# cchao0116/EasyDGL

Hardware: AMD Instinct MI355X
Metric: sequences/sec (fwd+bwd+Adam) B=512 L=100 d=128 |I|=20K (higher is better)
Workload: dtype bf16

## Files before the change

### easydgl_amd/_lib.py

```python
from __future__ import annotations

import ctypes
import os
from ctypes import c_char_p, c_float, c_int, c_int64, c_long, c_uint32, c_void_p

import torch

_HERE = os.path.dirname(os.path.abspath(__file__))
LIB_PATH = os.environ.get("EDGL_LIB_PATH") or os.path.join(_HERE, "libeasydgl_hip.so")

F32, BF16 = 0, 1
EPI_BIAS, EPI_GELU, EPI_SAVE_PRE, EPI_MUL_DGELU, EPI_ACCUM, EPI_OUT_F32, EPI_RELU = 1, 2, 4, 8, 16, 32, 64
MAU_CAUSAL, MAU_NO_DIAG, MAU_DIAG_ZERO = 1, 2, 4
MAU_NO_SKIP = 8
MAU_STREAM = 16
TATTN_CAUSAL = 1

P, I, F, L, U32, I64 = c_void_p, c_int, c_float, c_long, c_uint32, c_int64

SIGNATURES = {
    "edgl_last_error": (c_char_p, []),
    "edgl_version": (I, []),
    "edgl_profile_next": (I, [I, P, P]),
    "edgl_rng_advance": (I, [P, P]),
# ... 52 lines not shown
    "edgl_scatter_rows": (I, [P, P, I, I, P, I, P]),
    "edgl_score_lse_fwd": (I, [P, P, P, P, I, I, I, I, I, P, P, P, P, P, I, P]),
    "edgl_ce_loss_fwd": (I, [P, P, P, I, P, P, P]),
    "edgl_ce_loss_fwd_add": (I, [P, P, P, I, P, P, P, P, P]),
    "edgl_ce_loss_fwd_add_w": (I, [P, P, P, I, P, P, P, P, P, P]),
    "edgl_score_bwd_workspace": (L, [I, I, I, I, I]),
    "edgl_score_ce_bwd": (I, [P, P, P, P, P, P, P, I, I, I, I, I, P, P, P, P, P, I, P]),
    "edgl_score_flash_workspace": (L, [I, I, I, I, I]),
    "edgl_score_flash_fwd": (I, [P, P, P, P, I, I, I, I, I, P, P, P, P, I, P]),
    "edgl_score_prepare_table": (I, [P, I, I, I, I, I, P, I, P]),
    "edgl_score_flash_fwd_pre": (I, [P, P, P, P, I, I, I, I, I, P, P, P, P, I, I, P]),
    "edgl_score_flash_fwd_coef": (I, [P, P, P, P, I, I, I, P, P, P, P, P, I, P]),
    "edgl_score_flash_fwd_coef_w": (I, [P, P, P, P, I, I, I, P, P, P, P, P, P, I, P]),
    "edgl_score_flash_fwd_rows_w": (I, [P, P, P, P, I, I, I, P, P, P, P, P, P, P, P, I, P]),
    "edgl_score_ce_nparts": (I, [I, I]),
    "edgl_score_flash_fwd_rows_wp": (I, [P, P, P, P, I, I, I, P, P, P, P, P, P, P, P, P, I, P]),
    "edgl_ce_loss_parts": (I, [P, I, P, P, P, P, P]),
    "edgl_score_flash_bwd": (I, [P, P, P, P, P, P, P, I, I, I, I, I, P, P, P, P, P, I, P]),
    "edgl_score_flash_bwd_ex": (I, [P, P, P, P, P, P, P, I, I, I, I, I, P, P, P, P, P, I, I, P]),
    "edgl_score_flash_label_term": (I, [P, P, P, P, I, I, I, I, I, P, P, P, I, P]),
    "edgl_score_flash_label_term_det": (I, [P, P, P, P, I, I, I, I, I, P, P, P, P, I, P]),
    "edgl_reduce_defer": (I, [I, P]),
    "edgl_reduce_flush": (I, [P]),
    "edgl_mask_topk": (I, [P, I, I, I, P, I, I, P, P, P]),
    "edgl_score_topk_fused_supported": (I, [I, I, I, I, I, I]),
    "edgl_score_topk_fused_workspace": (L, [I, I, I, I, I]),
    "edgl_score_topk_fused": (I, [P, P, P, P, I, I, I, I, I, I, I, P, P, P, I, P]),
    "edgl_topk_merge": (I, [P, P, I, I, I, P, P, P]),
    "edgl_rank_metrics": (I, [P, I, I, P, P, P]),
    "edgl_tpp_workspace": (I, []),
    "edgl_tpp_fwd": (I, [P, P, P, P, P, I, I, I, I, I, F, P, P, I, P]),
    "edgl_tpp_bwd": (I, [P, P, P, P, P, I, I, I, I, I, F, P, P, P, P]),
    "edgl_tpp_fwd_bwd": (I, [P, P, P, P, P, I, I, I, I, I, F, P, P, I, P, P]),
    "edgl_tpp_norm": (I, [P, P, I, I, I, P, P]),
    "edgl_tpp_fwd_bwd_ex": (I, [P, P, P, P, P, I, I, I, I, I, F, P, P, I, P, I, P]),
    "edgl_tpp_rows_workspace": (L, [I, I, I]),
    "edgl_tpp_fwd_bwd_rows": (I, [P, P, P, P, P, I, I, I, I, I, F, P, P, I, P, P]),
    "edgl_tpp_prep_bytes": (L, [I, I, I]),
    "edgl_tpp_prep": (I, [P, P, P, P, I, I, I, I, P, P]),
    "edgl_bimau_bwd_tpp": (I, [P, P, P, P, P, P, P, I, P, F, P, P, P, I, I, I, I, I, F, P, U32, P, F, P, P, P, P, P, P, I, I, P]),
    "edgl_tpp_finish_parts": (I, [P, I, F, I, P, I, I, I, P, P, I, P]),
    "edgl_tpp_finish_parts_n": (I, [P, I, F, I, P, P, I, P]),
    "edgl_dp_counts": (I, [P, P, I, I, I, P, P]),
    "edgl_adam_step": (I, [P, P, P, P, L, F, F, F, F, P, F, P, I, P, P]),
    "edgl_step_begin": (I, [P, P, F, F, F, P]),
    "edgl_adam_apply": (I, [P, P, P, P, L, F, F, F, P, F, P, I, P, P]),
# ... 124 lines not shown
```

### easydgl_amd/build.py

```python
from __future__ import annotations

import hashlib
import os
import subprocess
import sys
from concurrent.futures import ThreadPoolExecutor

HERE = os.path.dirname(os.path.abspath(__file__))
CSRC = os.path.join(HERE, "csrc")
OUT = os.path.join(HERE, "libeasydgl_hip.so")
SOURCES = ["k_misc.hip", "k_data.hip", "k_encode.hip", "k_gemm.hip", "k_gemm2.hip", "k_layernorm.hip", "k_bimau_fwd.hip", "k_bimau_bwd.hip", "k_bimau_big.hip", "k_bimau_stream.hip",
           "k_score.hip", "k_score_strip.hip", "k_score_stripw.hip", "k_eval_topk.hip", "k_tattn.hip", "k_coding.hip", "k_tail.hip", "k_segsum.hip"]
HEADERS = ["edgl_common.h", "batch_prep.h", "score_plan.h", "topk_select.h", "gemm_tile.h", "bimau_common.h", "bimau_fwd_impl.h", "bimau_bwd_impl.h", os.path.join("..", "..", "include", "easydgl_hip.h")]
FLAGS = ["--offload-arch=gfx950", "-O3", "-std=c++17", "-fPIC", "-munsafe-fp-atomics", "-Wno-unused-result"]
EXTRA_FLAGS = {"k_bimau_fwd.hip": ["-mllvm", "-amdgpu-mfma-vgpr-form=1"],
               "k_bimau_bwd.hip": ["-mllvm", "-amdgpu-mfma-vgpr-form=1"],
               "k_bimau_big.hip": ["-mllvm", "-amdgpu-mfma-vgpr-form=1"],
               "k_bimau_stream.hip": ["-mllvm", "-amdgpu-mfma-vgpr-form=1"],
               "k_tattn.hip": ["-mllvm", "-amdgpu-mfma-vgpr-form=1"],
               "k_score_strip.hip": ["-fno-slp-vectorize", "-Wno-unused-value"] + (["-DSTRIP_SAFE"] if os.environ.get("EDGL_STRIP_SAFE") else []),
               "k_score_stripw.hip": ["-fno-slp-vectorize", "-Wno-unused-value"] + (["-DSTRIP_SAFE"] if os.environ.get("EDGL_STRIP_SAFE") else [])}


def _hipcc() -> str:
    for c in (os.environ.get("HIPCC"), "/opt/rocm/bin/hipcc", "hipcc"):
        if c and (os.path.isabs(c) and os.path.exists(c) or not os.path.isabs(c)):
            return c
    raise RuntimeError("hipcc not found")


def _digest(paths, extra=()) -> str:
    h = hashlib.sha256()
    for e in extra:
        h.update(str(e).encode() + b"\0")
    for p in paths:
        with open(p, "rb") as f:
# ... 56 lines not shown
```

### easydgl_amd/csrc/k_encode.hip

```cpp
#include "edgl_common.h"
#include "batch_prep.h"

namespace {

struct EncP {
    const int64_t* ids; const float* ts; const void* item_tab; const float* pos_tab; const float* mark_emb;
    const uint8_t* mark_table; const float* tscale;
    int B, T, C, E, I; int64_t mask_id; float time_scale;
    float rate; const uint64_t* rng; uint32_t stream_id;
    void* x0; float* spans; uint8_t* marks;
    int dhp, dht; float sq;
};

template <typename T>
__device__ __forceinline__ void encode_fwd_block(const EncP& p, long block) {
    const int cpr = p.C >> 3;
    const long gid = block * blockDim.x + threadIdx.x;
    const long row = gid / cpr;
    if (row >= (long)p.B * p.T) return;
    const int cv = (int)(gid % cpr), c0 = cv * 8, j0 = c0 >> 1;
    const int t = (int)(row % p.T);
    const int64_t id = p.ids[row];
    const int t1 = (t == 0) ? 1 : t;
    const long r1 = p.T > 1 ? row - t + t1 : row + 1;
// ... 96 lines not shown
};
template <typename T>
__global__ __launch_bounds__(256) void encode_prep_kernel(EncP p, PrepP q) {
    extern __shared__ __attribute__((aligned(16))) char prep_smem[];
    const int bid = (int)blockIdx.x;
    if (bid == 0) {
        batch_prep::compact_scan_body<256>(q.labels, q.R, q.perm, q.inv, q.nvalid, q.labels_c, reinterpret_cast<int*>(prep_smem));
    } else if (bid < q.nprep) {
        batch_prep::tpp_prep_sample(q.mpos, q.labels, q.ts_raw, p.mark_table, p.B, p.T, q.M, q.desc, bid - 1, prep_smem);
    } else {
        encode_fwd_block<T>(p, (long)(bid - q.nprep));
    }
}

struct EncBwdP {
    const int64_t* ids; const uint8_t* marks; const void* dx0;
    int B, T, C, E, I; float rate; const uint64_t* rng; uint32_t stream_id;
    float* d_item; float* part_pos; float* part_mk; int nchunk;
    int srows;
    const void* add1; const void* add2;
    float sq;
    const void* lab_rows; const int64_t* lab_ids; const float* lab_coef; const int32_t* lab_nvalid; int lab_R; int lab_blk0;
    float* d_bias;
    float* d_mark_zero;
};

template <typename T>
__global__ __launch_bounds__(256) void encode_bwd_kernel(EncBwdP p) {
    extern __shared__ float sm[];
    __shared__ float s_nm[64];
    const int t = blockIdx.x, chunk = blockIdx.y;
    if (t == 0 && chunk == 0 && p.d_mark_zero)
        for (int i = threadIdx.x; i < p.E * p.C; i += blockDim.x) p.d_mark_zero[i] = 0.f;
    const int bper = (p.B + p.nchunk - 1) / p.nchunk;
    const int b0 = chunk * bper, b1 = min(p.B, b0 + bper);
    const int cpr = p.C / 4, rows_par = 256 / cpr;
    const int cv = threadIdx.x % cpr, rl = threadIdx.x / cpr, c0 = cv * 4;
    const bool on = threadIdx.x < rows_par * cpr;
    const DropKey dk = make_dropkey(p.rng, p.stream_id, p.rate);
    float apos[4] = {0.f, 0.f, 0.f, 0.f}, amk[4] = {0.f, 0.f, 0.f, 0.f};
    for (int bb = b0; bb < b1; bb += 64) {
        __syncthreads();
        if (threadIdx.x < 64 && bb + threadIdx.x < b1) {
            const uint8_t* mrow = p.marks + ((long)(bb + threadIdx.x) * p.T + t) * p.E;
            int nm = 0;
            for (int e = 0; e < p.E; ++e) nm += mrow[e];
// ... 105 lines not shown
            float gv[4];
#pragma unroll
            for (int j = 0; j < 4; ++j) gv[j] = to_f32(g0.v[j]);
            drop_apply4(dk, (uint64_t)row * 3 * p.C + c0, gv);
#pragma unroll
            for (int j = 0; j < 4; ++j) atomicAdd(dst + j, sq * gv[j]);
        }
    }
    __syncthreads();
    for (int i = tid; i < SR * p.C; i += 256) {
        const int r = i / p.C, c = i % p.C;
        if (s_lead[r] == r && s_id[r] != 0) atomicAdd(p.d_item + (long)s_id[r] * p.C + c, acc[i]);
    }
}

typedef __attribute__((ext_vector_type(4))) short enc_s16x4;
__device__ __forceinline__ uint2 enc_tr_read(const bf16* tile, int ld, int k0, int z0, int lane) {
    const int G = lane >> 4, s = lane & 15;
    const bf16* p = tile + (k0 + 4 * G + (s >> 2)) * ld + z0 + 4 * (s & 3);
    enc_s16x4 v = __builtin_amdgcn_ds_read_tr16_b64_v4i16((__attribute__((address_space(3))) enc_s16x4*)p);
    return *reinterpret_cast<uint2*>(&v);
}
template <int CT>
__global__ __launch_bounds__(256) void encode_scatter_mfma_kernel(EncBwdP p) {
    constexpr int C = 16 * CT, LDG = C + 8, SR = SROWS;
    const int CF = p.C, coff = (int)blockIdx.y * C;
    __shared__ __attribute__((aligned(16))) bf16 Gs[SR * LDG];
    __shared__ __attribute__((aligned(16))) int s_id[SR];
    __shared__ __attribute__((aligned(16))) int s_lead[SR];
    const bool lab = p.lab_blk0 > 0 && (int)blockIdx.x >= p.lab_blk0;
    const long rows = lab ? (long)(p.lab_nvalid ? min(p.lab_R, p.lab_nvalid[0]) : p.lab_R) : (long)p.B * p.T;
    const long r0 = (long)((int)blockIdx.x - (lab ? p.lab_blk0 : 0)) * SR;
    if (lab && r0 >= rows) return;
    __shared__ float s_cf[SR], s_cb[SR];
    const int tid = threadIdx.x, lane = tid & 63, wave = tid >> 6, G = lane >> 4, g4 = G * 4, l15 = lane & 15;
    if (tid < SR) {
        const bool in = r0 + tid < rows;
        if (lab) {
            const float cf = in ? p.lab_coef[r0 + tid] : 0.f;
            s_id[tid] = (in && cf != 0.f) ? (int)p.lab_ids[r0 + tid] : 0;
            s_cf[tid] = cf;
            s_cb[tid] = 0.f;
        } else {
            s_id[tid] = in ? (int)p.ids[r0 + tid] : 0;
        }
    }
    constexpr int cpr = C / 4, rows_par = 256 / cpr, NR = SR / rows_par;
    const int cv = tid % cpr, rl = tid / cpr, c0 = cv * 4;
    const bf16* dx0 = reinterpret_cast<const bf16*>(lab ? p.lab_rows : p.dx0);
    const long ldrow = lab ? CF : 3 * CF;
    const bool adds = p.add1 && !lab;
    Frag4<bf16> g[NR], ga[NR], gb[NR];
#pragma unroll
    for (int k = 0; k < NR; ++k) {
        const long row = min(r0 + rl + (long)k * rows_par, rows - 1);
// ... 211 lines not shown
                                         const int32_t* lab_nvalid, int lab_R, float* d_bias, int dtype, void* stream) {
    EDGL_REQUIRE(lab_rows && lab_ids && lab_coef && d_bias && lab_R > 0, EDGL_ERR_NULL, "edgl_encode_bwd_add_label: null label operands");
    EDGL_REQUIRE(edgl_encode_bwd_label_fused(C, dtype) && (((uintptr_t)lab_rows | (uintptr_t)dx0 | (uintptr_t)add1 | (uintptr_t)add2) & 7) == 0,
                 EDGL_ERR_SHAPE, "edgl_encode_bwd_add_label: needs bf16, C %% 128 == 0 (or 64) and 8-byte aligned operands (C=%d)", C);
    return encode_bwd_impl(ids, marks, dx0, add1, add2, B, T, C, E, I, drop_rate, rng_state, stream_id, d_item, d_pos, d_mark_emb, workspace,
                           c_true, lab_rows, lab_ids, lab_coef, lab_nvalid, lab_R, d_bias, nullptr, dtype, stream);
}
static int encode_bwd_impl(const int64_t* ids, const uint8_t* marks, const void* dx0, const void* add1, const void* add2, int B,
                           int T, int C, int E, int I, float drop_rate, const uint64_t* rng_state, uint32_t stream_id,
                           float* d_item, float* d_pos, float* d_mark_emb, float* workspace, int c_true, const void* lab_rows,
                           const int64_t* lab_ids, const float* lab_coef, const int32_t* lab_nvalid, int lab_R, float* d_bias,
                           void* det_plan, int dtype, void* stream) {
    EDGL_REQUIRE(c_true >= 0 && c_true <= C, EDGL_ERR_SHAPE, "edgl_encode_bwd: true width %d exceeds C=%d", c_true, C);
    EDGL_REQUIRE((add1 == nullptr) == (add2 == nullptr), EDGL_ERR_NULL, "edgl_encode_bwd_add: add1 / add2 go together");
    EDGL_REQUIRE(ids && marks && dx0 && d_item && d_pos && d_mark_emb && workspace, EDGL_ERR_NULL,
                 "edgl_encode_bwd: null pointer");
    EDGL_REQUIRE(dtype == EDGL_F32 || dtype == EDGL_BF16, EDGL_ERR_DTYPE, "edgl_encode_bwd: bad dtype %d", dtype);
    EDGL_REQUIRE(C % 4 == 0 && C / 4 <= 256, EDGL_ERR_SHAPE, "edgl_encode_bwd: C=%d unsupported", C);
    float* part_pos = workspace;
    float* part_mk = workspace + (long)ENC_NCHUNK * T * C;
    int srows = SROWS;
    while (srows > 8 && (size_t)srows * C * sizeof(float) > 150 * 1024) srows >>= 1;
    EncBwdP p{ids, marks, dx0, B, T, C, E, I, drop_rate, rng_state, stream_id, d_item, part_pos, part_mk, ENC_NCHUNK, srows, add1, add2,
              sqrtf((float)(c_true > 0 ? c_true : C)), lab_rows, lab_ids, lab_coef, lab_nvalid, lab_R, 0, d_bias, d_mark_emb};
    hipStream_t st = (hipStream_t)stream;
    const int rows_par = 256 / (C / 4);
    dim3 grid(T, ENC_NCHUNK);
    const size_t smem = (size_t)rows_par * 2 * C * sizeof(float);
    if (dtype == EDGL_F32) hipLaunchKernelGGL((encode_bwd_kernel<float>), grid, dim3(256), smem, st, p);
    else hipLaunchKernelGGL((encode_bwd_kernel<bf16>), grid, dim3(256), smem, st, p);
    EDGL_LAUNCH_CHECK();
    if (det_plan) {
        const int rc = edgl_segsum_embed(ids, (long)B * T, C, I, dx0, add1, add2, p.sq, drop_rate, rng_state, stream_id, d_item, det_plan, dtype, st);
        if (rc) return rc;
    } else {
        const size_t smem_s = (size_t)srows * C * sizeof(float);
        EDGL_REQUIRE(smem_s <= 150 * 1024, EDGL_ERR_SHAPE, "edgl_encode_bwd: C=%d too large for the scatter stage", C);
        const unsigned nb = (unsigned)(((long)B * T + srows - 1) / srows);
        if (dtype == EDGL_BF16 && (C % 128 == 0 || C == 64) && (((uintptr_t)dx0 | (uintptr_t)add1 | (uintptr_t)add2) & 7) == 0) {
            unsigned nbm = (unsigned)(((long)B * T + SROWS - 1) / SROWS);
            if (lab_rows) { p.lab_blk0 = (int)nbm; nbm += (unsigned)((lab_R + SROWS - 1) / SROWS); }
            if (C % 128 == 0) hipLaunchKernelGGL((encode_scatter_mfma_kernel<8>), dim3(nbm, C / 128), dim3(256), 0, st, p);
            else hipLaunchKernelGGL((encode_scatter_mfma_kernel<4>), dim3(nbm), dim3(256), 0, st, p);
        } else if (dtype == EDGL_F32) {
            hipFuncSetAttribute((const void*)encode_scatter_kernel<float>, hipFuncAttributeMaxDynamicSharedMemorySize, (int)smem_s);
            hipLaunchKernelGGL((encode_scatter_kernel<float>), dim3(nb), dim3(256), smem_s, st, p);
        } else {
            hipFuncSetAttribute((const void*)encode_scatter_kernel<bf16>, hipFuncAttributeMaxDynamicSharedMemorySize, (int)smem_s);
            hipLaunchKernelGGL((encode_scatter_kernel<bf16>), dim3(nb), dim3(256), smem_s, st, p);
        }
        EDGL_LAUNCH_CHECK();
    }
    int rc = edgl_reduce_rows(part_pos, ENC_NCHUNK, T * C, (long)T * C, d_pos, 0, st);
    if (rc) return rc;
    if (E > 1) {
        rc = edgl_reduce_rows(part_mk, ENC_NCHUNK * T, C, C, d_mark_emb + C, 0, st);
        if (rc) return rc;
    }
    return EDGL_OK;
}
```

### easydgl_amd/csrc/k_misc.hip

```cpp
#include <cstdarg>
#include <cstdio>

#include "edgl_common.h"
#include "bimau_common.h"
#include "batch_prep.h"

namespace {
thread_local char g_err[512] = "";
constexpr int RED_BLOCKS = 256;
constexpr int SUMSQ_BLOCKS = 1024;
}

extern "C" void edgl_set_error(const char* fmt, ...) {
    va_list ap;
    va_start(ap, fmt);
    vsnprintf(g_err, sizeof(g_err), fmt, ap);
    va_end(ap);
}
extern "C" const char* edgl_last_error(void) { return g_err; }

namespace {
struct ProfSlot { int id = -1; hipEvent_t e0 = nullptr, e1 = nullptr; };
thread_local ProfSlot g_prof;
}
extern "C" int edgl_profile_next(int kernel_id, void* ev_start, void* ev_stop) {
    g_prof.id = kernel_id; g_prof.e0 = (hipEvent_t)ev_start; g_prof.e1 = (hipEvent_t)ev_stop;
    return EDGL_OK;
}
// ... 663 lines not shown
        float s = 0.f;
#pragma unroll
        for (int i = 0; i < 8; ++i) s += sm[i][tx];
        out[n] = accumulate ? out[n] + s : s;
    }
}

template <typename T>
__global__ void gelu_bwd_kernel(const T* dy, const T* pre, T* dz, long n) {
    for (long i = (long)blockIdx.x * blockDim.x + threadIdx.x; i < n; i += (long)gridDim.x * blockDim.x)
        dz[i] = from_f32<T>(to_f32(dy[i]) * dgelu_t<T>(to_f32(pre[i])));
}

template <typename T>
__global__ void relu_bwd_kernel(const T* dy, const T* y, T* dz, long n) {
    for (long i = (long)blockIdx.x * blockDim.x + threadIdx.x; i < n; i += (long)gridDim.x * blockDim.x)
        dz[i] = to_f32(y[i]) > 0.f ? dy[i] : from_f32<T>(0.f);
}

inline int grid_for(long n) { return (int)std::min<long>((n + 255) / 256, 4096); }

}

constexpr int RED_MAX_JOBS = 24;
constexpr int RED_COL_P = 32;
struct RedJob { const float* part; float* out; long ld; int P, N, blk0; };
struct RedBatch { RedJob j[RED_MAX_JOBS]; int n, blocks; };
static inline int red_blocks_scalar(const RedJob& j) { return (j.N + 31) / 32; }
static inline int red_blocks_vec(const RedJob& j) { return j.P <= RED_COL_P ? (j.N + 1023) / 1024 : (j.N + 31) / 32; }
thread_local bool g_red_defer = false;
thread_local RedBatch g_red_batch = {};

template <int RL>
__global__ __launch_bounds__(32 * RL) void reduce_rows_multi_kernel(RedBatch b) {
    __shared__ float sm[RL][33];
    int ji = 0;
    for (int i = 1; i < b.n; ++i)
        if ((int)blockIdx.x >= b.j[i].blk0) ji = i;
    const RedJob& jb = b.j[ji];
    const float* part = jb.part;
    const int P = jb.P, N = jb.N;
    const long ld = jb.ld;
    const int tx = threadIdx.x & 31, ty = threadIdx.x >> 5;
    const int n = ((int)blockIdx.x - jb.blk0) * 32 + tx;
    float a0 = 0.f, a1 = 0.f, a2 = 0.f, a3 = 0.f;
    if (n < N) {
        int p = ty;
        for (; p + 3 * RL < P; p += 4 * RL) {
            a0 += part[(long)p * ld + n];
            a1 += part[(long)(p + RL) * ld + n];
            a2 += part[(long)(p + 2 * RL) * ld + n];
            a3 += part[(long)(p + 3 * RL) * ld + n];
        }
        for (; p < P; p += RL) a0 += part[(long)p * ld + n];
    }
    sm[ty][tx] = (a0 + a1) + (a2 + a3);
    __syncthreads();
    if (ty == 0 && n < N) {
        float s = 0.f;
#pragma unroll
        for (int i = 0; i < RL; ++i) s += sm[i][tx];
        jb.out[n] = s;
    }
}

__global__ __launch_bounds__(256) void reduce_rows_multi_vec_kernel(RedBatch b) {
    __shared__ float4 sm[32][9];
    int ji = 0;
    for (int i = 1; i < b.n; ++i)
        if ((int)blockIdx.x >= b.j[i].blk0) ji = i;
    const RedJob& jb = b.j[ji];
    const int P = jb.P, N = jb.N;
    const long ld = jb.ld;
    if (P <= RED_COL_P) {
        const int n = (((int)blockIdx.x - jb.blk0) * 256 + (int)threadIdx.x) * 4;
        if (n >= N) return;
        const float* base = jb.part + n;
        float4 acc = make_float4(0.f, 0.f, 0.f, 0.f);
        int p0 = 0;
        for (; p0 + 8 <= P; p0 += 8) {
            float4 v[8];
#pragma unroll
            for (int u = 0; u < 8; ++u) v[u] = *reinterpret_cast<const float4*>(base + (long)(p0 + u) * ld);
#pragma unroll
            for (int u = 0; u < 8; ++u) { acc.x += v[u].x; acc.y += v[u].y; acc.z += v[u].z; acc.w += v[u].w; }
        }
        for (; p0 < P; ++p0) {
            const float4 v = *reinterpret_cast<const float4*>(base + (long)p0 * ld);
            acc.x += v.x; acc.y += v.y; acc.z += v.z; acc.w += v.w;
        }
        *reinterpret_cast<float4*>(jb.out + n) = acc;
        return;
    }
    const int tx = threadIdx.x & 7, ty = threadIdx.x >> 3;
    const int n = ((int)blockIdx.x - jb.blk0) * 32 + 4 * tx;
    float4 acc = make_float4(0.f, 0.f, 0.f, 0.f);
    if (n < N) {
        const float* base = jb.part + n;
        int p = ty;
        for (; p + 7 * 32 < P; p += 8 * 32) {
            float4 v[8];
#pragma unroll
            for (int u = 0; u < 8; ++u) v[u] = *reinterpret_cast<const float4*>(base + (long)(p + 32 * u) * ld);
#pragma unroll
            for (int u = 0; u < 8; ++u) { acc.x += v[u].x; acc.y += v[u].y; acc.z += v[u].z; acc.w += v[u].w; }
        }
        for (; p < P; p += 32) {
            const float4 v = *reinterpret_cast<const float4*>(base + (long)p * ld);
            acc.x += v.x; acc.y += v.y; acc.z += v.z; acc.w += v.w;
        }
    }
    sm[ty][tx] = acc;
    __syncthreads();
    if (ty < 4 && n < N) {
        float s = 0.f;
#pragma unroll
        for (int i = 0; i < 32; ++i) {
            const float4 v = sm[i][tx];
            s += ty == 0 ? v.x : (ty == 1 ? v.y : (ty == 2 ? v.z : v.w));
        }
        jb.out[n + ty] = s;
    }
}

int edgl_reduce_flush_impl(hipStream_t st) {
    if (g_red_batch.n == 0) return EDGL_OK;
    int maxp = 0;
    bool vec = true;
    for (int i = 0; i < g_red_batch.n; ++i) {
        const RedJob& j = g_red_batch.j[i];
        maxp = std::max(maxp, j.P);
        vec = vec && (j.N & 3) == 0 && (j.ld & 3) == 0 && (((uintptr_t)j.part | (uintptr_t)j.out) & 15) == 0;
    }
    int blocks = 0;
    for (int i = 0; i < g_red_batch.n; ++i) {
        RedJob& j = g_red_batch.j[i];
        j.blk0 = blocks;
        blocks += vec ? red_blocks_vec(j) : red_blocks_scalar(j);
    }
    g_red_batch.blocks = blocks;
    if (vec) hipLaunchKernelGGL(reduce_rows_multi_vec_kernel, dim3(g_red_batch.blocks), dim3(256), 0, st, g_red_batch);
    else if (maxp > 1024) hipLaunchKernelGGL(reduce_rows_multi_kernel<32>, dim3(g_red_batch.blocks), dim3(1024), 0, st, g_red_batch);
    else hipLaunchKernelGGL(reduce_rows_multi_kernel<8>, dim3(g_red_batch.blocks), dim3(256), 0, st, g_red_batch);
    g_red_batch.n = 0;
    g_red_batch.blocks = 0;
    EDGL_LAUNCH_CHECK();
    return EDGL_OK;
}

int edgl_reduce_rows(const float* part, int P, int N, long ld, float* out, int accumulate, hipStream_t st) {
    if (g_red_defer && !accumulate) {
        if (g_red_batch.n == RED_MAX_JOBS) {
            const int rc = edgl_reduce_flush_impl(st);
            if (rc) return rc;
        }
        RedJob& j = g_red_batch.j[g_red_batch.n++];
        j.part = part; j.out = out; j.ld = ld; j.P = P; j.N = N; j.blk0 = g_red_batch.blocks;
        g_red_batch.blocks += (N + 31) / 32;
        return EDGL_OK;
    }
    if (g_red_defer) {
        const int rc = edgl_reduce_flush_impl(st);
        if (rc) return rc;
    }
    hipLaunchKernelGGL(reduce_rows_kernel, dim3((N + 31) / 32), dim3(256), 0, st, part, P, N, ld, out, accumulate);
    EDGL_LAUNCH_CHECK();
    return EDGL_OK;
}

extern "C" int edgl_reduce_defer(int on, void* stream) {
    if (on < 0) {
        g_red_batch.n = 0;
        g_red_batch.blocks = 0;
        g_red_defer = false;
        return EDGL_OK;
    }
    if (!on && g_red_defer) {
        const int rc = edgl_reduce_flush_impl((hipStream_t)stream);
        if (rc) return rc;
    }
    g_red_defer = on != 0;
    return EDGL_OK;
}

extern "C" int edgl_reduce_flush(void* stream) { return edgl_reduce_flush_impl((hipStream_t)stream); }

extern "C" int edgl_rng_advance(uint64_t* rng_state, void* stream) {
    EDGL_REQUIRE(rng_state, EDGL_ERR_NULL, "edgl_rng_advance: null state");
    hipLaunchKernelGGL(rng_advance_kernel, dim3(1), dim3(1), 0, (hipStream_t)stream, rng_state);
    EDGL_LAUNCH_CHECK();
    return EDGL_OK;
}

// ... 380 lines not shown
```

### easydgl_amd/engine.py

```python
from __future__ import annotations

import ctypes
import os
from typing import Dict, Optional

import torch

from . import _lib, ops
from ._lib import check, lib
from .ops import _ptr, _stream

EPI_BIAS, EPI_GELU, EPI_SAVE_PRE, EPI_MUL_DGELU, EPI_ACCUM, EPI_OUT_F32 = 1, 2, 4, 8, 16, 32


class TrainEngine:
    _SIDE_STREAMS = {}

    def __init__(self, model, batch: int, use_graph: bool = True, process_group=None, fused_tail=None, flash_ce=None,
                 deterministic=None):
        env = os.environ.get
        self.sw_flash_ce = env("EDGL_FLASH_CE", "1") != "0"
        self.sw_tpp_fused = env("EDGL_TPP_FUSED", "1") != "0"
        self.sw_prep_in_encoder = env("EDGL_PREP_IN_ENCODER", "1") != "0"
        self.sw_bimau_order = env("EDGL_BIMAU_ORDER", "0") == "1"
        self.sw_ce_parts = env("EDGL_CE_PARTS", "1") != "0"
        self.sw_defer_loss = env("EDGL_DEFER_LOSS", "1") != "0"
        self.sw_adam_ex = env("EDGL_ADAM_EX", "1") != "0"
        self.sw_score_strip = env("EDGL_SCORE_STRIP", "1") != "0"
        self.m = model
        self.B = batch
        self.use_graph = use_graph
        self.deterministic = bool(getattr(model, "deterministic", False)) if deterministic is None else bool(deterministic)
        self.group = process_group
        self.graph: Optional[torch.cuda.CUDAGraph] = None
        m = model
        dev = m._arena.device
        self.dev = dev
        self.dt = m.act_dtype
        self.code = ops._DT[self.dt]
        B, T, C, H, E, M, I = batch, m.seqslen, m.num_units, m.num_heads, m.num_events, m.masklen, m.num_items
        self.T, self.C, self.H, self.E, self.M, self.I = T, C, H, E, M, I
        self.pad = tuple(m.pad)
        self.c_true = int(m.width_true) if self.pad[0] else 0
        self.qk_scale = float(m.qk_scale)
        gmax = int(lib.edgl_bimau_mark_group(C, H, self.code))
        if gmax <= 0:
            raise _lib.EdglError(f"TrainEngine: head dim {C // H} / {self.dt} unsupported by the attention kernels")
        self.mgroups = [(e0, min(E, e0 + gmax)) for e0 in range(0, E, gmax)] if E > gmax else []
        self.R = B * M
        self.rows = B * T
# ... 54 lines not shown
        self.nvalid = torch.zeros(1, device=dev, dtype=torch.int32)
        self.lse, self.lab_logit, self.coef = e(self.R, dtype=f32), e(self.R, dtype=f32), e(self.R, dtype=f32)
        self.loss = e(1, dtype=f32)
        self.ce_nparts = int(lib.edgl_score_ce_nparts(self.R, C)) if (self.flash_ce and self.sw_ce_parts) else 0
        self.ce_part = torch.zeros(self.ce_nparts + 1, device=dev, dtype=f32) if self.ce_nparts > 0 else None
        self.loss_aux, self.loss_tpp = torch.zeros(1, device=dev, dtype=f32), torch.zeros(1, device=dev, dtype=f32)
        self.ws_l2 = e(1024, dtype=f32)
        self.l2_nparts = int(lib.edgl_adam_l2_parts(m._arena.numel()))
        self.l2_parts = [torch.zeros(self.l2_nparts, device=dev, dtype=f32) for _ in range(2)] \
            if (m.l2_reg != 0.0 and not use_graph and not self.deterministic) else None
        self._l2p_cur, self._l2p_ready = 0, False
        key = (dev.type, dev.index if dev.index is not None else torch.cuda.current_device())
        if key not in TrainEngine._SIDE_STREAMS:
            TrainEngine._SIDE_STREAMS[key] = (torch.cuda.Stream(device=dev), torch.cuda.Stream(device=dev))
        self.side, self.side2 = TrainEngine._SIDE_STREAMS[key]
        self._pending_loss = None
        self.accumulate_loss = False
        self.loss_sum = torch.zeros(1, device=dev, dtype=torch.float64)
        self._pending_label = None
        self._lazy_loss, self._side_has_grads, self._loss_unjoined = False, False, False
        self._label_fused = False
        self.mau_flags = _lib.MAU_NO_SKIP
        self.adam_ex = (not use_graph) and self.sw_adam_ex and not self.deterministic
        self._rng_alt, self._adam_alt = torch.zeros_like(m._rng_state), torch.zeros_like(m._adam_state)
        self._slabs = None
        self._slab_info = None
        if self.adam_ex and self.flash_ce:
            info = (ctypes.c_long * 4)()
            check(lib.edgl_score_flash_slab_info(self.R, C, I, I, self.code, info), "edgl_score_flash_slab_info")
            self._slab_info = (int(info[0]), int(info[1]), int(info[2]))
        self._ar_events = None
        self.sync_loss = True
        self._deferred_loss = None
        self._alt = None
        if self.ce_part is not None:
            self._alt = dict(ce_part=torch.zeros_like(self.ce_part), loss_aux=torch.zeros_like(self.loss_aux),
                             tpp_desc=torch.zeros_like(self.tpp_desc) if self.tpp_desc is not None else None,
                             tpp_part=[torch.zeros_like(b["tpp_part"]) if b["tpp_part"] is not None else None for b in self.blk])
        self.counts = torch.zeros(2, device=dev, dtype=torch.int32)
        self._dp = False
        self.d_rows = e(self.R, C)
        self.plan_emb = ops.segsum_plan_buffer(self.rows, I, dev) if self.deterministic else None
        self.plan_lab = ops.segsum_plan_buffer(self.R, I, dev) if self.deterministic else None
        self.G1, self.G2, self.G3, self.G4 = e(B, T, C), e(B, T, C), e(B, T, C), e(B, T, C)
        self.G2c, self.G4c, self.G3c = e(B, T, 2 * C), e(B, T, 4 * C), e(B, T, 3 * C)
        wsz = [2 * self.R * lib.edgl_score_chunks(self.R, I),
# ... 364 lines not shown
                                             _ptr(att.scaling.grad),
                                             _ptr(self._ws(lib.edgl_bimau_bwd_workspace(B, T, C, H, E, code), torch.uint8)),
                                             _ptr(self.job_order), self.mau_flags, code, st), "edgl_bimau_bwd_ord")
            self._dense_dw(x_in, self.G4c, att.dense_kernel, att.dense_bias, cin, 4 * C)
            if self.fused_tail:
                check(lib.edgl_gemm_dw_defer(0, st), "edgl_gemm_dw_defer")
            d_in = self.G3c if i == 0 else self.G3
            self._dense_dx(self.G4c, att.dense_kernel, d_in, cin, 4 * C)
            if i == 0:
                self._issue_backward_end()
            if i > 0:
                check(lib.edgl_add_cols(_ptr(d_in), cin, _ptr(self.G1), _ptr(self.G2), C, self.rows, C, code, st), "edgl_add_cols")
                self.G2.copy_(self.G3)
                dY = self.G2
            else:
                dY = d_in
        d0 = drop(hd, 1)
        add1, add2 = (self.G1, self.G2) if self.blk else (None, None)
        if self.deterministic:
            check(lib.edgl_encode_bwd_add_det(_ptr(self.ids), _ptr(self.marks), _ptr(dY), _ptr(add1), _ptr(add2), B, T, C, E, I,
                                              float(d0.rate), d0.ptr(), d0.stream_id, _ptr(tab.grad), _ptr(m.pcoding.pembs.lookup_table.grad),
                                              _ptr(m.mark_embs.lookup_table.grad), _ptr(self._ws(lib.edgl_encode_bwd_workspace(B, T, C))),
                                              self.c_true, _ptr(self.plan_emb), code, st), "edgl_encode_bwd_add_det")
        elif self._label_fused:
            check(lib.edgl_encode_bwd_add_label(_ptr(self.ids), _ptr(self.marks), _ptr(dY), _ptr(add1), _ptr(add2), B, T, C, E, I,
                                                float(d0.rate), d0.ptr(), d0.stream_id, _ptr(tab.grad),
                                                _ptr(m.pcoding.pembs.lookup_table.grad), _ptr(m.mark_embs.lookup_table.grad),
                                                _ptr(self._ws(lib.edgl_encode_bwd_workspace(B, T, C))), self.c_true,
                                                _ptr(self.hrows_c), _ptr(lab), _ptr(self.coef), _ptr(self.nvalid), R,
                                                _ptr(m.output_bias.grad), code, st), "edgl_encode_bwd_add_label")
        else:
            check(lib.edgl_encode_bwd_add_ct(_ptr(self.ids), _ptr(self.marks), _ptr(dY), _ptr(add1), _ptr(add2), B, T, C, E, I,
                                             float(d0.rate), d0.ptr(), d0.stream_id, _ptr(tab.grad), _ptr(m.pcoding.pembs.lookup_table.grad),
                                             _ptr(m.mark_embs.lookup_table.grad), _ptr(self._ws(lib.edgl_encode_bwd_workspace(B, T, C))),
                                             self.c_true, code, st), "edgl_encode_bwd_add")

    def _issue_backward_end(self):
        m = self.m
        B, H = self.B, self.H
        pending, self._pending_loss = self._pending_loss, None

        def loss_launches(s, pending=pending, parts=[bj["tpp_part"] for bj in self.blk]):
            if self.fused_tpp:
                for j, bj in enumerate(self.blk):
                    check(lib.edgl_tpp_finish_parts_n(_ptr(parts[j]), B * H, float(m.ct_reg / H), H, _ptr(bj["tpp"]),
                                                      _ptr(self.loss_tpp), 1 if j > 0 else 0, s), "edgl_tpp_finish_parts")
            if pending is not None:
# ... 216 lines not shown
```

### include/easydgl_hip.h

```cpp
#ifndef EASYDGL_HIP_H
#define EASYDGL_HIP_H

#include <stdint.h>

#ifdef __cplusplus
extern "C" {
#endif

typedef enum { EDGL_F32 = 0, EDGL_BF16 = 1 } edgl_dtype;

enum {
    EDGL_OK = 0,
    EDGL_ERR_SHAPE = -1,
    EDGL_ERR_DTYPE = -2,
    EDGL_ERR_LAUNCH = -3,
    EDGL_ERR_NULL = -4,
    EDGL_ERR_WORKSPACE = -5
};

enum {
    EDGL_EPI_BIAS = 1,
    EDGL_EPI_GELU = 2,
    EDGL_EPI_SAVE_PRE = 4,
    EDGL_EPI_MUL_DGELU = 8,
// ... 216 lines not shown
int edgl_score_ce_nparts(int R, int C);
int edgl_score_flash_fwd_rows_wp(const void* rows, const void* table, const float* out_bias, const int64_t* labels, int R, int C,
                                 int I, const int32_t* nvalid, const int32_t* wtotal, const float* gscale, float* row_lse,
                                 float* label_logit, float* coef, void* d_rows, float* ce_part, float* workspace, int dtype,
                                 void* stream);
int edgl_ce_loss_parts(const float* ce_part, int nparts, float* loss_out, const float* add_in, const float* add_in2,
                       const int32_t* wtotal, void* stream);
int edgl_score_flash_bwd(const void* rows, const void* table, const float* out_bias, const int64_t* labels,
                         const float* row_lse, const float* coef, const float* gscale, int R, int C, int I, int i0,
                         int i1, const int32_t* nvalid, void* d_rows, float* d_table, float* d_bias, float* workspace,
                         int dtype, void* stream);
int edgl_score_flash_bwd_ex(const void* rows, const void* table, const float* out_bias, const int64_t* labels,
                            const float* row_lse, const float* coef, const float* gscale, int R, int C, int I, int i0,
                            int i1, const int32_t* nvalid, void* d_rows, float* d_table, float* d_bias, float* workspace,
                            int defer_label_term, int dtype, void* stream);
int edgl_score_flash_label_term(const void* rows, const int64_t* labels, const float* coef, const float* gscale, int R, int C, int I,
                                int i0, int i1, const int32_t* nvalid, float* d_table, float* d_bias, int dtype, void* stream);
int edgl_score_flash_label_term_det(const void* rows, const int64_t* labels, const float* coef, const float* gscale, int R, int C,
                                    int I, int i0, int i1, const int32_t* nvalid, float* d_table, float* d_bias, void* plan, int dtype,
                                    void* stream);

int edgl_reduce_defer(int on, void* stream);
int edgl_reduce_flush(void* stream);

int edgl_tpp_workspace(void);
int edgl_tpp_fwd(const float* lam, const int64_t* masked_pos, const int64_t* labels, const float* ts_raw,
                 const uint8_t* mark_table, int B, int T, int H, int E, int M, float coef, float* sums,
                 float* reg_out, int accumulate, void* stream);
int edgl_tpp_bwd(const float* lam, const int64_t* masked_pos, const int64_t* labels, const float* ts_raw,
                 const uint8_t* mark_table, int B, int T, int H, int E, int M, float coef,
                 const float* sums, const float* gscale, float* d_lam, void* stream);
int edgl_tpp_fwd_bwd(const float* lam, const int64_t* masked_pos, const int64_t* labels, const float* ts_raw,
                     const uint8_t* mark_table, int B, int T, int H, int E, int M, float coef, float* sums,
                     float* reg_out, int accumulate, float* d_lam, void* stream);
int edgl_tpp_norm(const int64_t* labels, const uint8_t* mark_table, int B, int M, int E, float* sums, void* stream);
int edgl_tpp_fwd_bwd_ex(const float* lam, const int64_t* masked_pos, const int64_t* labels, const float* ts_raw,
                        const uint8_t* mark_table, int B, int T, int H, int E, int M, float coef, float* sums,
                        float* reg_out, int accumulate, float* d_lam, int with_norm, void* stream);
long edgl_tpp_rows_workspace(int B, int H, int M);
int edgl_tpp_fwd_bwd_rows(const float* lam, const int64_t* masked_pos, const int64_t* labels, const float* ts_raw,
                          const uint8_t* mark_table, int B, int T, int H, int E, int M, float coef, float* sums,
                          float* reg_out, int accumulate, float* d_lam, void* stream);

int edgl_dp_counts(const int64_t* labels, const uint8_t* mark_table, int B, int M, int E, int32_t* counts, void* stream);
long edgl_tpp_prep_bytes(int B, int T, int M);
int edgl_tpp_prep(const int64_t* masked_pos, const int64_t* labels, const float* ts_raw, const uint8_t* mark_table, int B, int T,
// ... 125 lines not shown
```

Measured before the change: 673,200.

## Fold deferred partial-sum reductions into the encode scatter kernel launch

Deferred row-reduction jobs, plus the encoder's own position and mark partial reductions, are appended as extra workgroups of the MFMA encode-scatter kernel. Those workgroups run the shared vectorised reduction body and use the kernel's shared row buffer as scratch. This removes separate reduction kernel launches and lets the reduction overlap with the scatter. In exchange, the grid is larger and an overlap check is needed so no reduction writes into buffers the scatter updates. It applies only when defer is on, the path is non-deterministic, and C is at most 128.

```diff
diff --git a/easydgl_amd/_lib.py b/easydgl_amd/_lib.py
--- a/easydgl_amd/_lib.py
+++ b/easydgl_amd/_lib.py
@@ -98,6 +98,8 @@
     "edgl_score_flash_label_term_det": (I, [P, P, P, P, I, I, I, I, I, P, P, P, P, I, P]),
     "edgl_reduce_defer": (I, [I, P]),
     "edgl_reduce_flush": (I, [P]),
+    "edgl_reduce_partials": (I, [P, I, I, L, P, I, P]),
+    "edgl_reduce_ride": (I, [I]),
     "edgl_mask_topk": (I, [P, I, I, I, P, I, I, P, P, P]),
     "edgl_score_topk_fused_supported": (I, [I, I, I, I, I, I]),
     "edgl_score_topk_fused_workspace": (L, [I, I, I, I, I]),
diff --git a/easydgl_amd/build.py b/easydgl_amd/build.py
--- a/easydgl_amd/build.py
+++ b/easydgl_amd/build.py
@@ -11,7 +11,7 @@
 OUT = os.path.join(HERE, "libeasydgl_hip.so")
 SOURCES = ["k_misc.hip", "k_data.hip", "k_encode.hip", "k_gemm.hip", "k_gemm2.hip", "k_layernorm.hip", "k_bimau_fwd.hip", "k_bimau_bwd.hip", "k_bimau_big.hip", "k_bimau_stream.hip",
            "k_score.hip", "k_score_strip.hip", "k_score_stripw.hip", "k_eval_topk.hip", "k_tattn.hip", "k_coding.hip", "k_tail.hip", "k_segsum.hip"]
-HEADERS = ["edgl_common.h", "batch_prep.h", "score_plan.h", "topk_select.h", "gemm_tile.h", "bimau_common.h", "bimau_fwd_impl.h", "bimau_bwd_impl.h", os.path.join("..", "..", "include", "easydgl_hip.h")]
+HEADERS = ["edgl_common.h", "batch_prep.h", "score_plan.h", "topk_select.h", "gemm_tile.h", "bimau_common.h", "bimau_fwd_impl.h", "bimau_bwd_impl.h", "red_batch.h", os.path.join("..", "..", "include", "easydgl_hip.h")]
 FLAGS = ["--offload-arch=gfx950", "-O3", "-std=c++17", "-fPIC", "-munsafe-fp-atomics", "-Wno-unused-result"]
 EXTRA_FLAGS = {"k_bimau_fwd.hip": ["-mllvm", "-amdgpu-mfma-vgpr-form=1"],
                "k_bimau_bwd.hip": ["-mllvm", "-amdgpu-mfma-vgpr-form=1"],
diff --git a/easydgl_amd/csrc/k_encode.hip b/easydgl_amd/csrc/k_encode.hip
--- a/easydgl_amd/csrc/k_encode.hip
+++ b/easydgl_amd/csrc/k_encode.hip
@@ -1,5 +1,6 @@
 #include "edgl_common.h"
 #include "batch_prep.h"
+#include "red_batch.h"
 
 namespace {
 
@@ -142,6 +143,7 @@
     float sq;
     const void* lab_rows; const int64_t* lab_ids; const float* lab_coef; const int32_t* lab_nvalid; int lab_R; int lab_blk0;
     float* d_bias;
+    int red_blk0;
     float* d_mark_zero;
 };
 
@@ -293,15 +295,21 @@
     return *reinterpret_cast<uint2*>(&v);
 }
 template <int CT>
-__global__ __launch_bounds__(256) void encode_scatter_mfma_kernel(EncBwdP p) {
+__global__ __launch_bounds__(256) void encode_scatter_mfma_kernel(EncBwdP p, RedBatch rb) {
     constexpr int C = 16 * CT, LDG = C + 8, SR = SROWS;
     const int CF = p.C, coff = (int)blockIdx.y * C;
     __shared__ __attribute__((aligned(16))) bf16 Gs[SR * LDG];
     __shared__ __attribute__((aligned(16))) int s_id[SR];
     __shared__ __attribute__((aligned(16))) int s_lead[SR];
-    const bool lab = p.lab_blk0 > 0 && (int)blockIdx.x >= p.lab_blk0;
+    if ((int)blockIdx.x >= p.red_blk0 && (int)blockIdx.x < p.red_blk0 + rb.blocks) {
+        static_assert(sizeof(Gs) >= 32 * 9 * sizeof(float4), "the reduction's scratch lives in the row image");
+        reduce_rows_vec_block(rb, (int)blockIdx.x - p.red_blk0, reinterpret_cast<float4(*)[9]>(Gs));
+        return;
+    }
+    const int bx = (int)blockIdx.x - (p.red_blk0 == 0 ? rb.blocks : 0);
+    const bool lab = p.lab_blk0 > 0 && bx >= p.lab_blk0;
     const long rows = lab ? (long)(p.lab_nvalid ? min(p.lab_R, p.lab_nvalid[0]) : p.lab_R) : (long)p.B * p.T;
-    const long r0 = (long)((int)blockIdx.x - (lab ? p.lab_blk0 : 0)) * SR;
+    const long r0 = (long)(bx - (lab ? p.lab_blk0 : 0)) * SR;
     if (lab && r0 >= rows) return;
     __shared__ float s_cf[SR], s_cb[SR];
     const int tid = threadIdx.x, lane = tid & 63, wave = tid >> 6, G = lane >> 4, g4 = G * 4, l15 = lane & 15;
@@ -559,7 +567,7 @@
     int srows = SROWS;
     while (srows > 8 && (size_t)srows * C * sizeof(float) > 150 * 1024) srows >>= 1;
     EncBwdP p{ids, marks, dx0, B, T, C, E, I, drop_rate, rng_state, stream_id, d_item, part_pos, part_mk, ENC_NCHUNK, srows, add1, add2,
-              sqrtf((float)(c_true > 0 ? c_true : C)), lab_rows, lab_ids, lab_coef, lab_nvalid, lab_R, 0, d_bias, d_mark_emb};
+              sqrtf((float)(c_true > 0 ? c_true : C)), lab_rows, lab_ids, lab_coef, lab_nvalid, lab_R, 0, d_bias, 0, d_mark_emb};
     hipStream_t st = (hipStream_t)stream;
     const int rows_par = 256 / (C / 4);
     dim3 grid(T, ENC_NCHUNK);
@@ -567,6 +575,8 @@
     if (dtype == EDGL_F32) hipLaunchKernelGGL((encode_bwd_kernel<float>), grid, dim3(256), smem, st, p);
     else hipLaunchKernelGGL((encode_bwd_kernel<bf16>), grid, dim3(256), smem, st, p);
     EDGL_LAUNCH_CHECK();
+    const RedJob own[2] = {{part_pos, d_pos, (long)T * C, ENC_NCHUNK, T * C, 0}, {part_mk, E > 1 ? d_mark_emb + C : d_mark_emb, (long)C, ENC_NCHUNK * T, C, 0}};
+    bool rode = false;
     if (det_plan) {
         const int rc = edgl_segsum_embed(ids, (long)B * T, C, I, dx0, add1, add2, p.sq, drop_rate, rng_state, stream_id, d_item, det_plan, dtype, st);
         if (rc) return rc;
@@ -577,8 +587,21 @@
         if (dtype == EDGL_BF16 && (C % 128 == 0 || C == 64) && (((uintptr_t)dx0 | (uintptr_t)add1 | (uintptr_t)add2) & 7) == 0) {
             unsigned nbm = (unsigned)(((long)B * T + SROWS - 1) / SROWS);
             if (lab_rows) { p.lab_blk0 = (int)nbm; nbm += (unsigned)((lab_R + SROWS - 1) / SROWS); }
-            if (C % 128 == 0) hipLaunchKernelGGL((encode_scatter_mfma_kernel<8>), dim3(nbm, C / 128), dim3(256), 0, st, p);
-            else hipLaunchKernelGGL((encode_scatter_mfma_kernel<4>), dim3(nbm), dim3(256), 0, st, p);
+            RedBatch rb;
+            rb.n = rb.blocks = 0;
+            if (C <= 128) {
+                int first = 1;
+                const int nred = edgl_reduce_ride_take(own, E > 1 ? 2 : 1, d_item, d_item + (long)I * C, d_bias, d_bias ? d_bias + (I - 1) : d_bias,
+                                                       &rb, &first, st);
+                if (nred < 0) return nred;
+                if (nred > 0) {
+                    rode = true;
+                    p.red_blk0 = first ? 0 : (int)nbm;
+                    nbm += (unsigned)nred;
+                }
+            }
+            if (C % 128 == 0) hipLaunchKernelGGL((encode_scatter_mfma_kernel<8>), dim3(nbm, C / 128), dim3(256), 0, st, p, rb);
+            else hipLaunchKernelGGL((encode_scatter_mfma_kernel<4>), dim3(nbm), dim3(256), 0, st, p, rb);
         } else if (dtype == EDGL_F32) {
             hipFuncSetAttribute((const void*)encode_scatter_kernel<float>, hipFuncAttributeMaxDynamicSharedMemorySize, (int)smem_s);
             hipLaunchKernelGGL((encode_scatter_kernel<float>), dim3(nb), dim3(256), smem_s, st, p);
@@ -588,10 +611,8 @@
         }
         EDGL_LAUNCH_CHECK();
     }
-    int rc = edgl_reduce_rows(part_pos, ENC_NCHUNK, T * C, (long)T * C, d_pos, 0, st);
-    if (rc) return rc;
-    if (E > 1) {
-        rc = edgl_reduce_rows(part_mk, ENC_NCHUNK * T, C, C, d_mark_emb + C, 0, st);
+    for (int i = 0; i < (E > 1 ? 2 : 1) && !rode; ++i) {
+        const int rc = edgl_reduce_rows(own[i].part, own[i].P, own[i].N, own[i].ld, own[i].out, 0, st);
         if (rc) return rc;
     }
     return EDGL_OK;
diff --git a/easydgl_amd/csrc/k_misc.hip b/easydgl_amd/csrc/k_misc.hip
--- a/easydgl_amd/csrc/k_misc.hip
+++ b/easydgl_amd/csrc/k_misc.hip
@@ -4,6 +4,7 @@
 #include "edgl_common.h"
 #include "bimau_common.h"
 #include "batch_prep.h"
+#include "red_batch.h"
 
 namespace {
 thread_local char g_err[512] = "";
@@ -713,14 +714,14 @@
 
 }
 
-constexpr int RED_MAX_JOBS = 24;
-constexpr int RED_COL_P = 32;
-struct RedJob { const float* part; float* out; long ld; int P, N, blk0; };
-struct RedBatch { RedJob j[RED_MAX_JOBS]; int n, blocks; };
 static inline int red_blocks_scalar(const RedJob& j) { return (j.N + 31) / 32; }
 static inline int red_blocks_vec(const RedJob& j) { return j.P <= RED_COL_P ? (j.N + 1023) / 1024 : (j.N + 31) / 32; }
+static inline bool red_job_vec(const RedJob& j) {
+    return (j.N & 3) == 0 && (j.ld & 3) == 0 && (((uintptr_t)j.part | (uintptr_t)j.out) & 15) == 0;
+}
 thread_local bool g_red_defer = false;
 thread_local RedBatch g_red_batch = {};
+thread_local int g_red_ride = 0;
 
 template <int RL>
 __global__ __launch_bounds__(32 * RL) void reduce_rows_multi_kernel(RedBatch b) {
@@ -757,61 +758,7 @@
 
 __global__ __launch_bounds__(256) void reduce_rows_multi_vec_kernel(RedBatch b) {
     __shared__ float4 sm[32][9];
-    int ji = 0;
-    for (int i = 1; i < b.n; ++i)
-        if ((int)blockIdx.x >= b.j[i].blk0) ji = i;
-    const RedJob& jb = b.j[ji];
-    const int P = jb.P, N = jb.N;
-    const long ld = jb.ld;
-    if (P <= RED_COL_P) {
-        const int n = (((int)blockIdx.x - jb.blk0) * 256 + (int)threadIdx.x) * 4;
-        if (n >= N) return;
-        const float* base = jb.part + n;
-        float4 acc = make_float4(0.f, 0.f, 0.f, 0.f);
-        int p0 = 0;
-        for (; p0 + 8 <= P; p0 += 8) {
-            float4 v[8];
-#pragma unroll
-            for (int u = 0; u < 8; ++u) v[u] = *reinterpret_cast<const float4*>(base + (long)(p0 + u) * ld);
-#pragma unroll
-            for (int u = 0; u < 8; ++u) { acc.x += v[u].x; acc.y += v[u].y; acc.z += v[u].z; acc.w += v[u].w; }
-        }
-        for (; p0 < P; ++p0) {
-            const float4 v = *reinterpret_cast<const float4*>(base + (long)p0 * ld);
-            acc.x += v.x; acc.y += v.y; acc.z += v.z; acc.w += v.w;
-        }
-        *reinterpret_cast<float4*>(jb.out + n) = acc;
-        return;
-    }
-    const int tx = threadIdx.x & 7, ty = threadIdx.x >> 3;
-    const int n = ((int)blockIdx.x - jb.blk0) * 32 + 4 * tx;
-    float4 acc = make_float4(0.f, 0.f, 0.f, 0.f);
-    if (n < N) {
-        const float* base = jb.part + n;
-        int p = ty;
-        for (; p + 7 * 32 < P; p += 8 * 32) {
-            float4 v[8];
-#pragma unroll
-            for (int u = 0; u < 8; ++u) v[u] = *reinterpret_cast<const float4*>(base + (long)(p + 32 * u) * ld);
-#pragma unroll
-            for (int u = 0; u < 8; ++u) { acc.x += v[u].x; acc.y += v[u].y; acc.z += v[u].z; acc.w += v[u].w; }
-        }
-        for (; p < P; p += 32) {
-            const float4 v = *reinterpret_cast<const float4*>(base + (long)p * ld);
-            acc.x += v.x; acc.y += v.y; acc.z += v.z; acc.w += v.w;
-        }
-    }
-    sm[ty][tx] = acc;
-    __syncthreads();
-    if (ty < 4 && n < N) {
-        float s = 0.f;
-#pragma unroll
-        for (int i = 0; i < 32; ++i) {
-            const float4 v = sm[i][tx];
-            s += ty == 0 ? v.x : (ty == 1 ? v.y : (ty == 2 ? v.z : v.w));
-        }
-        jb.out[n + ty] = s;
-    }
+    reduce_rows_vec_block(b, (int)blockIdx.x, sm);
 }
 
 int edgl_reduce_flush_impl(hipStream_t st) {
@@ -821,7 +768,7 @@
     for (int i = 0; i < g_red_batch.n; ++i) {
         const RedJob& j = g_red_batch.j[i];
         maxp = std::max(maxp, j.P);
-        vec = vec && (j.N & 3) == 0 && (j.ld & 3) == 0 && (((uintptr_t)j.part | (uintptr_t)j.out) & 15) == 0;
+        vec = vec && red_job_vec(j);
     }
     int blocks = 0;
     for (int i = 0; i < g_red_batch.n; ++i) {
@@ -859,7 +806,50 @@
     return EDGL_OK;
 }
 
+int edgl_reduce_ride_take(const RedJob* own, int nown, const float* lo0, const float* hi0, const float* lo1, const float* hi1,
+                          RedBatch* out, int* first_blocks, hipStream_t st) {
+    if (!g_red_defer || !g_red_ride) return 0;
+    auto rides = [&](const RedJob& j) {
+        const float* o0 = j.out;
+        const float* o1 = j.out + j.N;
+        return red_job_vec(j) && !(o0 < hi0 && lo0 < o1) && !(o0 < hi1 && lo1 < o1);
+    };
+    for (int i = 0; i < g_red_batch.n; ++i)
+        if (!rides(g_red_batch.j[i])) return 0;
+    for (int i = 0; i < nown; ++i)
+        if (!rides(own[i])) return 0;
+    if (g_red_batch.n + nown > RED_MAX_JOBS) {
+        const int rc = edgl_reduce_flush_impl(st);
+        if (rc) return rc;
+    }
+    for (int i = 0; i < nown; ++i) g_red_batch.j[g_red_batch.n++] = own[i];
+    int blocks = 0;
+    for (int i = 0; i < g_red_batch.n; ++i) {
+        g_red_batch.j[i].blk0 = blocks;
+        blocks += red_blocks_vec(g_red_batch.j[i]);
+    }
+    g_red_batch.blocks = blocks;
+    *out = g_red_batch;
+    *first_blocks = g_red_ride == 1;
+    g_red_batch.n = 0;
+    g_red_batch.blocks = 0;
+    return blocks;
+}
+
+extern "C" int edgl_reduce_ride(int on) {
+    EDGL_REQUIRE(on >= 0 && on <= 2, EDGL_ERR_SHAPE, "edgl_reduce_ride: on = %d (0: off, 1: in front of the scatter's workgroups, 2: behind)", on);
+    g_red_ride = on;
+    return EDGL_OK;
+}
+
+extern "C" int edgl_reduce_partials(const float* part, int P, int N, long ld, float* out, int accumulate, void* stream) {
+    EDGL_REQUIRE(part && out, EDGL_ERR_NULL, "edgl_reduce_partials: null pointer");
+    EDGL_REQUIRE(P > 0 && N > 0 && ld >= N, EDGL_ERR_SHAPE, "edgl_reduce_partials: bad shape P=%d N=%d ld=%ld", P, N, ld);
+    return edgl_reduce_rows(part, P, N, ld, out, accumulate, (hipStream_t)stream);
+}
+
 extern "C" int edgl_reduce_defer(int on, void* stream) {
+    if (on <= 0) g_red_ride = 0;
     if (on < 0) {
         g_red_batch.n = 0;
         g_red_batch.blocks = 0;
diff --git a/easydgl_amd/csrc/red_batch.h b/easydgl_amd/csrc/red_batch.h
--- /dev/null
+++ b/easydgl_amd/csrc/red_batch.h
@@ -0,0 +1,68 @@
+#pragma once
+#include "edgl_common.h"
+
+constexpr int RED_MAX_JOBS = 24;
+constexpr int RED_COL_P = 32;
+struct RedJob { const float* part; float* out; long ld; int P, N, blk0; };
+struct RedBatch { RedJob j[RED_MAX_JOBS]; int n, blocks; };
+
+int edgl_reduce_ride_take(const RedJob* own, int nown, const float* lo0, const float* hi0, const float* lo1, const float* hi1,
+                          RedBatch* out, int* first_blocks, hipStream_t st);
+
+__device__ __forceinline__ void reduce_rows_vec_block(const RedBatch& b, int bid, float4 (*sm)[9]) {
+    int ji = 0;
+    for (int i = 1; i < b.n; ++i)
+        if (bid >= b.j[i].blk0) ji = i;
+    const RedJob& jb = b.j[ji];
+    const int P = jb.P, N = jb.N;
+    const long ld = jb.ld;
+    if (P <= RED_COL_P) {
+        const int n = ((bid - jb.blk0) * 256 + (int)threadIdx.x) * 4;
+        if (n >= N) return;
+        const float* base = jb.part + n;
+        float4 acc = make_float4(0.f, 0.f, 0.f, 0.f);
+        int p0 = 0;
+        for (; p0 + 8 <= P; p0 += 8) {
+            float4 v[8];
+#pragma unroll
+            for (int u = 0; u < 8; ++u) v[u] = *reinterpret_cast<const float4*>(base + (long)(p0 + u) * ld);
+#pragma unroll
+            for (int u = 0; u < 8; ++u) { acc.x += v[u].x; acc.y += v[u].y; acc.z += v[u].z; acc.w += v[u].w; }
+        }
+        for (; p0 < P; ++p0) {
+            const float4 v = *reinterpret_cast<const float4*>(base + (long)p0 * ld);
+            acc.x += v.x; acc.y += v.y; acc.z += v.z; acc.w += v.w;
+        }
+        *reinterpret_cast<float4*>(jb.out + n) = acc;
+        return;
+    }
+    const int tx = threadIdx.x & 7, ty = threadIdx.x >> 3;
+    const int n = (bid - jb.blk0) * 32 + 4 * tx;
+    float4 acc = make_float4(0.f, 0.f, 0.f, 0.f);
+    if (n < N) {
+        const float* base = jb.part + n;
+        int p = ty;
+        for (; p + 7 * 32 < P; p += 8 * 32) {
+            float4 v[8];
+#pragma unroll
+            for (int u = 0; u < 8; ++u) v[u] = *reinterpret_cast<const float4*>(base + (long)(p + 32 * u) * ld);
+#pragma unroll
+            for (int u = 0; u < 8; ++u) { acc.x += v[u].x; acc.y += v[u].y; acc.z += v[u].z; acc.w += v[u].w; }
+        }
+        for (; p < P; p += 32) {
+            const float4 v = *reinterpret_cast<const float4*>(base + (long)p * ld);
+            acc.x += v.x; acc.y += v.y; acc.z += v.z; acc.w += v.w;
+        }
+    }
+    sm[ty][tx] = acc;
+    __syncthreads();
+    if (ty < 4 && n < N) {
+        float s = 0.f;
+#pragma unroll
+        for (int i = 0; i < 32; ++i) {
+            const float4 v = sm[i][tx];
+            s += ty == 0 ? v.x : (ty == 1 ? v.y : (ty == 2 ? v.z : v.w));
+        }
+        jb.out[n + ty] = s;
+    }
+}
diff --git a/easydgl_amd/engine.py b/easydgl_amd/engine.py
--- a/easydgl_amd/engine.py
+++ b/easydgl_amd/engine.py
@@ -26,6 +26,8 @@
         self.sw_ce_parts = env("EDGL_CE_PARTS", "1") != "0"
         self.sw_defer_loss = env("EDGL_DEFER_LOSS", "1") != "0"
         self.sw_adam_ex = env("EDGL_ADAM_EX", "1") != "0"
+        self.sw_reduce_ride = env("EDGL_REDUCE_RIDE", "1") != "0"
+        self.sw_reduce_ride_behind = env("EDGL_REDUCE_RIDE", "1") == "2"
         self.sw_score_strip = env("EDGL_SCORE_STRIP", "1") != "0"
         self.m = model
         self.B = batch
@@ -126,6 +128,7 @@
         self._label_fused = False
         self.mau_flags = _lib.MAU_NO_SKIP
         self.adam_ex = (not use_graph) and self.sw_adam_ex and not self.deterministic
+        self.reduce_ride = self.sw_reduce_ride and not self.deterministic
         self._rng_alt, self._adam_alt = torch.zeros_like(m._rng_state), torch.zeros_like(m._adam_state)
         self._slabs = None
         self._slab_info = None
@@ -536,7 +539,10 @@
                                               float(d0.rate), d0.ptr(), d0.stream_id, _ptr(tab.grad), _ptr(m.pcoding.pembs.lookup_table.grad),
                                               _ptr(m.mark_embs.lookup_table.grad), _ptr(self._ws(lib.edgl_encode_bwd_workspace(B, T, C))),
                                               self.c_true, _ptr(self.plan_emb), code, st), "edgl_encode_bwd_add_det")
-        elif self._label_fused:
+            return
+        if self.reduce_ride:
+            check(lib.edgl_reduce_ride(2 if self.sw_reduce_ride_behind else 1), "edgl_reduce_ride")
+        if self._label_fused:
             check(lib.edgl_encode_bwd_add_label(_ptr(self.ids), _ptr(self.marks), _ptr(dY), _ptr(add1), _ptr(add2), B, T, C, E, I,
                                                 float(d0.rate), d0.ptr(), d0.stream_id, _ptr(tab.grad),
                                                 _ptr(m.pcoding.pembs.lookup_table.grad), _ptr(m.mark_embs.lookup_table.grad),
diff --git a/include/easydgl_hip.h b/include/easydgl_hip.h
--- a/include/easydgl_hip.h
+++ b/include/easydgl_hip.h
@@ -262,6 +262,8 @@
 
 int edgl_reduce_defer(int on, void* stream);
 int edgl_reduce_flush(void* stream);
+int edgl_reduce_partials(const float* part, int P, int N, long ld, float* out, int accumulate, void* stream);
+int edgl_reduce_ride(int on);
 
 int edgl_tpp_workspace(void);
 int edgl_tpp_fwd(const float* lam, const int64_t* masked_pos, const int64_t* labels, const float* ts_raw,
```

Result: faster. 680,000, median of 6 (+1.0%).
